# karenyang/GCN-VAE

Measured on AMD Instinct MI355X. Metric: edges/sec R-GCN forward+backward, FB15k-237 emb=200, higher is better.
Workload: dtype f32; 1 GPU; FB15k-237-shaped synthetic full graph (BASELINE configs[1]): 14541 entities, 474 directed relation types, E=544230 directed edges on this rank (544230 in the trained graph), 2-layer R-GCN-VAE bdd num_bases=100 emb_dim=200 dropout 0.2, 0 IAF blocks, DistMult decoder on T=220000 triplets per rank, step = fwd + loss(BCE+reg+KL+MMD) + bwd + clip + Adam; edges_per_gpu=544230, trained_graph_edges=544230, nodes=14541, triplets_per_gpu=220000, n_flows=0, gemm_precision=f32, launch=hipgraph, parallelism=single GPU, optimizer=replicated clip + Adam, k1_operands=f32

## Files before the change

gcn-vae_amd/csrc/k_loss.hip:

```cpp
#include "common.h"

namespace gv {

constexpr int RED_BLOCKS = 1024;

__device__ __forceinline__ float block_sum_256(float v, float* sm ) {
    v = wave_sum(v);
    const int lane = threadIdx.x & 63, w = threadIdx.x >> 6;
    __syncthreads();
    if (lane == 0) sm[w] = v;
    __syncthreads();
    return sm[0] + sm[1] + sm[2] + sm[3];
}

__global__ __launch_bounds__(256) void k_final_sum(const float* part, int n, float scale, float* out, int accumulate) {
    __shared__ float sm[4];
    float acc = 0.f;
    for (int i = threadIdx.x; i < n; i += 256) acc += part[i];
    const float tot = block_sum_256(acc, sm);
    if (threadIdx.x == 0) *out = accumulate ? *out + scale * tot : scale * tot;
}

__global__ __launch_bounds__(256) void k_loss_combine(const float* p0, int n0, float s0, const float* p1, int n1, float s1,
                                                      const float* p2, int n2, float s2, const float* p3, int n3, float s3,
// ... 1019 lines not shown
    for (int i = blockIdx.x * 256 + threadIdx.x; i < total; i += gridDim.x * 256) {
        const int j = i / h, c = i - j * h;
        const float raw = z_pre[(size_t)(k + j) * h + c];
        const float v = softplus_t(raw) + 1e-8f;
        float gm = 0.f, gs = 0.f;
        for (int r = j; r < s; r += k) {
            gm += g[(size_t)r * h + c];
            gs += g[(size_t)r * h + c] * eps[(size_t)r * h + c];
        }
        const float gr = gs * 0.5f / sqrtf(v) * (raw > 20.f ? 1.f : 1.f / (1.f + expf(-raw)));
        gz_pre[i] = accumulate ? gz_pre[i] + gm : gm;
        gz_pre[total + i] = accumulate ? gz_pre[total + i] + gr : gr;
    }
}

struct DmFusedParams {
    const int4* items;
    int n_items;
    const int* rel_s;
    const int* rel_o;
    const int* rel_tid;
    const float* e;
    int ld_e;
    const float* w;
    int ld_w;
    const float* labels;
    const float* bias;
    const int* pos3;
    float* score;
    float* delta;
// ... 518 lines not shown
extern "C" int gv_prior_sample_fwd(const float* z_pre, const float* eps, float* out, int s, int k, int h, void* stream) {
    GV_REQUIRE(z_pre && eps && out, GV_ERR_NULL, "gv_prior_sample_fwd: NULL pointer");
    GV_REQUIRE(s > 0 && k > 0 && h > 0, GV_ERR_SHAPE, "gv_prior_sample_fwd: bad shape");
    hipLaunchKernelGGL(k_prior_sample_fwd, dim3((s * h + 255) / 256), dim3(256), 0, GV_ST, z_pre, eps, out, s, k, h);
    return launch_status("gv_prior_sample_fwd");
}

extern "C" int gv_prior_sample_bwd(const float* z_pre, const float* eps, const float* g, float* gz_pre, int accumulate,
                                   int s, int k, int h, void* stream) {
    GV_REQUIRE(z_pre && eps && g && gz_pre, GV_ERR_NULL, "gv_prior_sample_bwd: NULL pointer");
    GV_REQUIRE(s > 0 && k > 0 && h > 0, GV_ERR_SHAPE, "gv_prior_sample_bwd: bad shape");
    hipLaunchKernelGGL(k_prior_sample_bwd, dim3((k * h + 255) / 256), dim3(256), 0, GV_ST, z_pre, eps, g, gz_pre, accumulate, s, k, h);
    return launch_status("gv_prior_sample_bwd");
}

extern "C" int gv_distmult_bce_fwd_grad(const int32_t* items, int n_items, const int32_t* rel_s, const int32_t* rel_o,
                                        const int32_t* rel_tid, const float* embed, int ld_e, const float* w_rel, int ld_w,
                                        const float* labels, const float* bias, const int32_t* pos3, float* score,
                                        float* delta, float* u, float* partial, float* workspace, int64_t t, int h,
                                        void* stream) {
    GV_REQUIRE(items && rel_s && rel_o && rel_tid && embed && w_rel && labels && score && delta && u && workspace,
               GV_ERR_NULL, "gv_distmult_bce_fwd_grad: NULL pointer");
    GV_REQUIRE(t > 0 && t < (1ll << 30) && n_items > 0, GV_ERR_SHAPE, "gv_distmult_bce_fwd_grad: t=%lld n_items=%d",
               (long long)t, n_items);
    GV_REQUIRE(h > 0 && h <= 256 && h % 4 == 0 && ld_e >= h && ld_w >= h && ld_e % 4 == 0 && ld_w % 4 == 0, GV_ERR_SHAPE,
               "gv_distmult_bce_fwd_grad: h=%d (ld %d, %d): the fused sweep covers h <= 256, h %% 4 == 0", h, ld_e, ld_w);
    GV_REQUIRE(aligned16(embed) && aligned16(w_rel) && aligned16(u) && aligned16(partial), GV_ERR_ALIGN,
               "gv_distmult_bce_fwd_grad: 16-B alignment required");
    DmFusedParams p{(const int4*)items, n_items, rel_s, rel_o, rel_tid, embed, ld_e, w_rel, ld_w, labels, bias, pos3,
                    score, delta, u, partial, workspace, h};
// ... 27 lines not shown
```

gcn-vae_amd/encoders.py:

```python
import random

import numpy as np
import torch
import torch.nn as nn
import torch.nn.functional as F

from . import ops, prob
from .flows import MADE, PermuteLayer
from .layers import RelGraphConv


class EmbeddingLayer(ops.StayOnDevice, nn.Module):
    def __init__(self, num_nodes, h_dim):
        super().__init__()
        self.embedding = nn.Embedding(num_nodes, h_dim)

    def forward(self, g, h, r, norm):
        h = ops.to_module_device(self.embedding.weight, h)
        return ops.embedding(self.embedding.weight, h.squeeze(), ops.device_rng(self.embedding.weight.device),
                             sole_consumer=True)


class DistLayer(ops.StayOnDevice, nn.Module):

# ... 57 lines not shown
        idx = torch.distributions.categorical.Categorical(self.pi).sample((batch,))
        x = prob.sample_gaussian(m[idx], v[idx])
        if self.n_flows > 0:
            for flow in self.nf[::-1]:
                x, _ = flow.inverse(x)
        return x

    def compute_kernel(self, x, y):
        dim = x.size(1)
        d2 = (x.unsqueeze(1) - y.unsqueeze(0)).pow(2).mean(2) / float(dim)
        return torch.exp(-d2)

    def get_kl(self, z):
        return ops.kl_to_mixture(z, self.z_mean, self.z_sigma, self.z_pre.squeeze(0), self.flow_log_prob)

    def _prior_draw(self, device, dtype):
        num_sample = 200
        rows = (num_sample // self.k) * self.k if num_sample // self.k > 1 else self.k
        if self.mmd_eps_override is not None:
            eps = self.mmd_eps_override
        elif self._prior_eps_next is not None:
            eps, self._prior_eps_next = self._prior_eps_next, None
        else:
            eps = torch.empty(rows, self.h_dim, device=device, dtype=dtype)
            ops.device_rng(device).fill([(eps, ops.RNG_NORMAL, 0.0, self.rng_stream_prior)])
        return ops.prior_sample(self.z_pre.squeeze(0), eps)

    def _prior_rows(self):
        num_sample = 200
        return (num_sample // self.k) * self.k if num_sample // self.k > 1 else self.k

    def _draw_noise(self, n, device):
        jobs, eps = [], self.eps_override
        for layer in (self.rconv_layer_1, self.rconv_layer_2):
            if layer.wants_keep_mask():
                layer._keep_next = torch.empty(n, layer.out_feat, dtype=torch.uint8, device=device)
                jobs.append(layer.keep_job(layer._keep_next))
        if eps is None:
            eps = torch.empty(n, self.h_dim, dtype=torch.float32, device=device)
            jobs.append((eps, ops.RNG_NORMAL, 0.0, self.rng_stream_eps))
        if self.batch_mmd_prior_with_forward and self.training and self.mmd_eps_override is None:
            self._prior_eps_next = torch.empty(self._prior_rows(), self.h_dim, dtype=torch.float32, device=device)
            jobs.append((self._prior_eps_next, ops.RNG_NORMAL, 0.0, self.rng_stream_prior))
        if jobs:
            ops.device_rng(device).fill(jobs)
        return eps

    def mmd_inputs(self, z):
        num_sample = 200
        if self._z_pri_flowed is not None:
            z_pri, self._z_pri_flowed = self._z_pri_flowed, None
        else:
            z_pri = self._prior_draw(z.device, z.dtype)
            if self.n_flows > 0:
                for flow in self.nf:
                    z_pri, _ = flow.forward(z_pri)
        if self.mmd_index_override is not None:
            pick = self.mmd_index_override
        elif self.row_part is not None and getattr(self.row_part, 'real_positions', None) is not None:
            real = self.row_part.real_positions
            pick = torch.as_tensor(real[random.sample(range(len(real)), num_sample)], device=z.device)
        else:
            pick = torch.tensor(random.sample(range(z.shape[0]), num_sample), device=z.device)
        return z_pri, pick

    def get_mmd(self, z):
        z_pri, pick = self.mmd_inputs(z)
        return ops.mmd(z_pri, ops.embedding(z, pick))
# ... 176 lines not shown
```

gcn-vae_amd/lib.py:

```python
import ctypes
import os

import torch

_HERE = os.path.dirname(os.path.abspath(__file__))
LIB_PATH = os.path.join(_HERE, 'libgcnvae_hip.so')

_P, _I, _L, _F = ctypes.c_void_p, ctypes.c_int, ctypes.c_int64, ctypes.c_float

SIGNATURES = {
    'gv_version': (_I, []),
    'gv_last_error_string': (ctypes.c_char_p, []),
    'gv_index_caps': (None, [_L, _I, _I, _P, _P, _P]),
    'gv_index_workspace_bytes': (_L, [_L, _I]),
    'gv_build_csr': (_I, [_P, _L, _I, _I, _P, _P, _P, _I, _P, _I, _P, _L, _P]),
    'gv_build_csr_batch_workspace_bytes': (_L, [_P, _I]),
    'gv_build_csr_batch': (_I, [_P, _I, _P, _L, _P]),
    'gv_triplet_lists': (_I, [_P, _I, _L, _P, _P, _P, _P, _P, _P, _P, _P, _P]),
    'gv_widen2_i32': (_I, [_P, _P, _L, _P, _P, _L, _P]),
    'gv_graph_index_build': (_I, [_P, _P, _L, _I, _I, _I, _I, _P, _P, _P, _P, _I, _P, _I, _P, _P, _P, _P, _I, _P, _I, _P, _L, _P]),
    'gv_relation_index_build': (_I, [_P, _P, _P, _P, _P, _L, _I, _I, _P, _P, _P, _P, _P, _P, _P, _I, _P, _I, _P, _L, _P]),
    'gv_triplet_index_build': (_I, [_P, _L, _I, _I, _I, _I, _P, _P, _P, _P, _P, _I, _P, _I, _P, _P, _P, _P, _P, _I, _P, _I,
                                    _P, _L, _P]),
    'gv_perm_sample': (_I, [_L, _L, ctypes.c_uint64, ctypes.c_uint64, _P, _P, ctypes.c_uint32, _P, _P]),
# ... 126 lines not shown
    'gv_mean_sq2': (_I, [_P, _L, _F, _P, _L, _F, _P, _P, _P, _L, _P]),
    'gv_axpby': (_I, [_L, _P, _F, _P, _F, _P, _P]),
    'gv_mul': (_I, [_L, _P, _P, _P, _P]),
    'gv_mul_multi': (_I, [_I, _P, _P, _P, _P, _P]),
    'gv_kl_workspace_bytes': (_L, [_L, _I, _I]),
    'gv_kl_fwd': (_I, [_P, _P, _I, _P, _P, _P, _P, _P, _P, _L, _I, _I, _P, _P]),
    'gv_kl_bwd': (_I, [_P, _P, _I, _P, _P, _P, _P, _F, _F, _P, _P, _P, _P, _I, _P, _I, _L, _I, _I, _P, _P]),
    'gv_reparam_kl_fwd': (_I, [_P, _P, _P, _P, _P, _P, _P, _P, _L, _I, _I, _P]),
    'gv_reparam_kl_bwd': (_I, [_P, _P, _P, _P, _P, _P, _P, _F, _F, _P, _P, _P, _I, _P, _L, _I, _I, _P]),
    'gv_loss_combine': (_I, [_P, _L, _P, _L, _L, _P, _L, _I, _I, _P, _I, _I, _F, _F, _F, _P, _P, _P, _P]),
    'gv_lincomb4': (_I, [_P, _F, _P, _F, _P, _F, _P, _F, _P, _P]),
    'gv_mmd_fwd': (_I, [_P, _P, _P, _I, _I, _I, _P, _P, _P]),
    'gv_mmd_bwd': (_I, [_P, _P, _P, _I, _I, _I, _P, _F, _P, _P, _P]),
    'gv_prior_sample_fwd': (_I, [_P, _P, _P, _I, _I, _I, _P]),
    'gv_prior_sample_bwd': (_I, [_P, _P, _P, _P, _I, _I, _I, _I, _P]),
    'gv_iaf_update_fwd': (_I, [_P, _P, _I, _P, _P, _P, _L, _I, _P]),
    'gv_iaf_update_bwd': (_I, [_P, _P, _I, _P, _P, _P, _P, _P, _P, _L, _I, _P]),
    'gv_iaf_update_bwd_acc': (_I, [_P, _P, _I, _P, _P, _P, _P, _I, _P, _P, _L, _I, _P]),
    'gv_rowsum': (_I, [_P, _I, _I, _I, _P, _L, _P]),
    'gv_reverse_cols': (_I, [_P, _P, _L, _I, _P]),
    'gv_mean_rows_multi': (_I, [_I, _P, _L, _P, _P, _P, _P]),
    'gv_mean_rows_bwd': (_I, [_P, _L, _L, _P, _P, _P]),
    'gv_adam_step': (_I, [_P, _P, _P, _P, _L, _P, _F, _F, _F, _F, _F, _P, _P]),
    'gv_clip_adam_step': (_I, [_P, _P, _P, _P, _L, _P, _P, _F, _F, _F, _F, _F, _P, _I, _P]),
}

_lib = None
_fns = {}


# ... 61 lines not shown
```

gcn-vae_amd/ops.py:

```python
import contextlib
import ctypes as _ct
import itertools as _it
import os as _os
from dataclasses import dataclass
from typing import Optional

import torch

from . import lib
from .lib import ptr

ACT_NONE, ACT_RELU = 0, 1

DIRECT_GRAD = {}
GRAD_FRESH = set()
DIRECT_EPOCH = [0]


def _stamp_direct(ctx):
    ctx._gv_direct_epoch = DIRECT_EPOCH[0]


def _verify_direct(ctx):
    if getattr(ctx, '_gv_direct_epoch', DIRECT_EPOCH[0]) != DIRECT_EPOCH[0]:
# ... 2533 lines not shown
        z_pre, eps = ctx.saved_tensors
        if g is None:
            return None, None
        g = _chk(g.contiguous(), name='g')
        d_zp = _direct_flat(z_pre)
        gz = d_zp if d_zp is not None else torch.empty_like(z_pre)
        lib.call('gv_prior_sample_bwd', ptr(z_pre), ptr(eps), ptr(g), ptr(gz), 1 if d_zp is not None else 0, eps.shape[0],
                 z_pre.shape[0] // 2, z_pre.shape[1], lib.stream())
        return (None if d_zp is not None else gz), None


def prior_sample(z_pre, eps):
    return _PriorSample.apply(z_pre, eps)


class _LossHead(torch.autograd.Function):

    @staticmethod
    def forward(ctx, z, z_mean, z_sigma, w_rel, z_pre, flp, z_pri, pick, labels, tidx, reg_w, kl_w, mmd_w, score_bias,
                embed_rows=None, rows_dev=None, kl_link=None, grad_mode=True):
        z, ld_z = _row_major(z, 'embed')
        if rows_dev is not None:
            rows_dev = _chk(rows_dev.reshape(-1), torch.int32, 'rows_dev')
            if kl_w <= 0 or embed_rows is not None:
                raise NotImplementedError('rows_dev needs kl_w > 0 (the padding rows are masked in the KL pass) and no embed_rows')
        w_rel, ld_w = _row_major(w_rel, 'w_relation')
        labels = _chk(labels.reshape(-1), name='labels')
        dev, (n, h), T = z.device, z.shape, tidx.T
        if labels.numel() != T:
            raise ValueError('labels / triplets length mismatch')
        f32 = dict(dtype=torch.float32, device=dev)
        ctx.set_materialize_grads(False)
        scal = torch.empty(4, **f32)
        pred, reg, kl, mmd = scal[0:1], scal[1:2], scal[2:3], scal[3:4]
        ws, ws2 = torch.empty(2048, **f32), torch.empty(1024, **f32)
        score = torch.empty(T, **f32)
        loss = torch.empty((), **f32)
        bias = flp if (score_bias and flp is not None) else None
        resp = wsk = z_post = wsm = None
        link = kl_link if (kl_link is not None and not kl_link.claimed and kl_w > 0 and flp is None and rows_dev is None
                           and embed_rows is None and kl_link.matches(z_pre) and kl_link.resp.shape[0] == n) else None
        if link is not None:
            link.claimed = True
        if kl_w > 0:
            z_mean, z_sigma = _chk(z_mean.contiguous(), name='z_mean'), _chk(z_sigma.contiguous(), name='z_sigma')
            z_pre = _chk(z_pre.contiguous(), name='z_pre')
            k = z_pre.shape[0] // 2
            if link is None:
                wsk = torch.empty(int(lib.load().gv_kl_workspace_bytes(n, h, k)) // 4, **f32)
                resp = torch.empty(n, k, **f32)
        if mmd_w > 0:
            z_pri = _chk(z_pri.contiguous(), name='z_pri')
            pick = _chk(pick.reshape(-1), torch.int64, 'pick')
            wsm = torch.empty(z_pri.shape[0] + pick.numel(), **f32)
        if ld_z != h or ld_w != h:
            raise ValueError('loss_head needs contiguous embeddings and relation table')
        st = lib.stream()
        if link is not None:
            resp, wsk = link.resp, link.ws
        elif kl_w > 0:
            lib.call('gv_kl_fwd', ptr(z), ptr(z_mean), h, ptr(z_sigma), ptr(z_pre), ptr(flp), ptr(resp), None, ptr(wsk),
                     n, h, k, ptr(rows_dev), st)
        if mmd_w > 0:
            lib.call('gv_mmd_fwd', ptr(z_pri), ptr(z), ptr(pick), z_pri.shape[0], pick.numel(), h, None, ptr(wsm), st)
        z_count = z.numel() if embed_rows is None else int(embed_rows) * h
        lib.call('gv_mean_sq2', ptr(z), z.numel(), 1.0 / z_count, ptr(w_rel), w_rel.numel(), 1.0 / w_rel.numel(), None,
                 ptr(ws2), ptr(rows_dev), n, st)
        ctx.fused = None
        if grad_mode and (ctx.needs_input_grad[0] or ctx.needs_input_grad[3]) and distmult_fused_ok(z, ld_z, w_rel, ld_w):
            ctx.fused = _distmult_fused_fwd(z, ld_z, w_rel, ld_w, labels, bias, tidx, score, ws)
            ctx.ws = ws
        else:
            lib.call('gv_distmult_bce_fwd', ptr(z), ld_z, ptr(w_rel), ld_w, ptr(tidx.trip32), ptr(tidx.fwd_order), ptr(labels),
                     ptr(bias), ptr(score), None, ptr(ws), T, h, st)
        lib.call('gv_loss_combine', ptr(ws), T, ptr(ws2), z.numel(), w_rel.numel(), ptr(wsk) if kl_w > 0 else None, n, h,
                 (z_pre.shape[0] // 2) if kl_w > 0 else 0, ptr(wsm) if mmd_w > 0 else None,
                 z_pri.shape[0] if mmd_w > 0 else 0, pick.numel() if mmd_w > 0 else 0, float(reg_w), float(kl_w),
                 float(mmd_w), ptr(scal), ptr(loss), ptr(rows_dev), st)
        ctx.save_for_backward(z, z_mean if kl_w > 0 else None, z_sigma if kl_w > 0 else None, w_rel,
                              z_pre if kl_w > 0 else None, resp, z_pri if mmd_w > 0 else None, z_post,
                              pick if mmd_w > 0 else None, labels, score, wsk, rows_dev)
        ctx.meta = (tidx, float(reg_w), float(kl_w), float(mmd_w), bias is not None, flp is not None and kl_w > 0)
        ctx.z_count = z_count
        ctx.kl_link = link
        ctx.direct_w = _direct(w_rel) if ld_w == h else None
        _stamp_direct(ctx)
        out_pred, out_kl, out_mmd = pred.reshape(()), kl.reshape(1), mmd.reshape(())
        ctx.mark_non_differentiable(out_pred, out_kl, out_mmd)
        return loss, out_pred, out_kl, out_mmd

    @staticmethod
    def backward(ctx, g, _gp, _gk, _gm):
        if g is None:
            return (None,) * 18
        z, z_mean, z_sigma, w_rel, z_pre, resp, z_pri, z_post, pick, labels, score, wsk, rows_dev = ctx.saved_tensors
        z_count = ctx.z_count
        tidx, reg_w, kl_w, mmd_w, has_bias, flp_in_kl = ctx.meta
        dev, (n, h), T = z.device, z.shape, tidx.T
        f32 = dict(dtype=torch.float32, device=dev)
        g = _chk(g.reshape(1).contiguous(), name='gloss')
        fused = ctx.fused
        dscore = torch.empty(T, **f32) if fused is None else None
        dbias = torch.empty((), **f32) if has_bias else None
        ws = torch.empty(1024, **f32) if fused is None else None
        link = ctx.kl_link
        gz = torch.empty_like(z) if link is None else None
        gm = gv = gzp = d_zp = g_pri = g_post = None
        if link is not None:
            link.gkl, link.gscale, link.z_extra = g, kl_w, 2.0 * reg_w / z_count
            d_zp = True
        elif kl_w > 0:
            k = z_pre.shape[0] // 2
            d_zp = _direct_flat(z_pre)
            gm, gv = torch.empty_like(z), torch.empty_like(z)
            gzp = d_zp if d_zp is not None else torch.empty_like(z_pre)
        if mmd_w > 0:
            g_pri = torch.empty_like(z_pri)
        _verify_direct(ctx)
        d_w = ctx.direct_w
        g_w = d_w if d_w is not None else torch.empty_like(w_rel)
        g_flp = torch.empty((), **f32) if (has_bias or flp_in_kl) else None
        st = lib.stream()
        with fork(1):
            s1 = lib.stream()
            if link is not None:
                pass
            elif kl_w > 0:
                lib.call('gv_kl_bwd', ptr(z), ptr(z_mean), h, ptr(z_sigma), ptr(z_pre), ptr(resp), ptr(g), kl_w,
                         2.0 * reg_w / z_count, ptr(gz), ptr(gm), ptr(gv), ptr(gzp), 1 if d_zp is not None else 0, ptr(wsk),
                         1, n, h, k, ptr(rows_dev), s1)
            else:
                lib.call('gv_axpby', z.numel(), ptr(g), 2.0 * reg_w / z_count, ptr(z), 0.0, ptr(gz), s1)
            if mmd_w > 0 and link is None:
                lib.call('gv_mmd_bwd', ptr(z_pri), ptr(z), ptr(pick), z_pri.shape[0], pick.numel(), h, ptr(g), mmd_w,
                         ptr(g_pri), ptr(gz), s1)
        if fused is not None:
            d_inc = _distmult_fused_finish(fused, g, tidx, w_rel, h, 2.0 * reg_w / w_rel.numel(), g_w, d_w is not None, ctx.ws,
                                           dbias)
            idx_inc = None if tidx.pos3 is not None else tidx.inc_tid
        else:
            if tidx.pos3 is not None:
                d_inc, d_rel, idx_inc, idx_rel = torch.empty(2 * T, **f32), torch.empty(T, **f32), None, None
            else:
                d_inc, d_rel, idx_inc, idx_rel = dscore, dscore, tidx.inc_tid, tidx.rel_tid
            lib.call('gv_bce_grad', ptr(score), ptr(labels), ptr(g), ptr(dscore), ptr(tidx.pos3),
                     ptr(d_inc) if tidx.pos3 is not None else None, ptr(d_rel) if tidx.pos3 is not None else None,
                     ptr(dbias), ptr(ws), T, st)
            bdd_grad_weight(tidx.rel, tidx.rel_s, tidx.rel_o, d_rel, idx_rel, z, z, h, 1, 1, out=g_w,
                            accumulate=d_w is not None)
            lib.call('gv_axpby', w_rel.numel(), ptr(g), 2.0 * reg_w / w_rel.numel(), ptr(w_rel), 1.0, ptr(g_w), st)
        join(1)
        g_z = bdd_aggregate(indices.largest_first(tidx.inc) if indices.K1_ITEMS_LARGEST_FIRST else tidx.inc, tidx.inc_other, tidx.inc_rel,
                            d_inc, idx_inc, z, w_rel, h, 1, 1, addend=gz)
        if link is not None and mmd_w > 0:
            lib.call('gv_mmd_bwd', ptr(z_pri), ptr(z), ptr(pick), z_pri.shape[0], pick.numel(), h, ptr(g), mmd_w,
                     ptr(g_pri), ptr(g_z), st)
        if g_flp is not None:
            lib.call('gv_lincomb4', ptr(dbias) if has_bias else None, 1.0, ptr(g) if flp_in_kl else None, kl_w, None, 0.0,
                     None, 0.0, ptr(g_flp), st)
        return (g_z, gm, gv, (None if d_w is not None else g_w), (None if d_zp is not None else gzp), g_flp, g_pri, None,
                None, None, None, None, None, None, None, None, None, None)


def loss_head(z, z_mean, z_sigma, w_rel, z_pre, flp, z_pri, pick, labels, tidx, reg_w, kl_w, mmd_w, score_bias,
              embed_rows=None, rows_dev=None):
    return _LossHead.apply(z, z_mean, z_sigma, w_rel, z_pre, flp, z_pri, pick, labels, tidx, float(reg_w), float(kl_w),
                           float(mmd_w), bool(score_bias), embed_rows, rows_dev, getattr(z, '_gv_kl_link', None),
                           torch.is_grad_enabled())


from .made import *
from .made import _ChainLayer, _RowLayer, _MADEForward, _MADEForwardBF16
from . import made


TRANSE_MAX_DIM = 512


def _i32(t, name, n=None):
    t = _chk(t, torch.int32, name)
    if not t.is_contiguous() or (n is not None and t.numel() != n):
        raise ValueError(f'{name}: expected a contiguous int32 tensor of {n} entries')
    return t
# ... 364 lines not shown
```

gcn-vae_amd/train.py:

```python
import argparse
import time

import numpy as np
import torch
import torch.nn as nn

from . import ops, ranking, sampling
from .optim import FlatAdam
from .data import load_data
from .encoders import KGVAE, RGCN
from .sampling import node_norm_to_edge_norm


class LinkPredict(ops.StayOnDevice, nn.Module):
    def __init__(self, model_class, in_dim, h_dim, num_rels, num_bases=-1, num_hidden_layers=1, dropout=0,
                 use_cuda=True, reg_param=0, kl_param=0, mmd_param=0, k=1, n_flows=0):
        super().__init__()
        self.encoder = model_class(num_nodes=in_dim, h_dim=h_dim, out_dim=h_dim, num_rels=num_rels * 2,
                                   num_bases=num_bases, num_hidden_layers=num_hidden_layers, dropout=dropout,
                                   use_self_loop=use_cuda, use_cuda=use_cuda, k=k, n_flows=n_flows)
        self.reg_param, self.kl_param, self.mmd_param = reg_param, kl_param, mmd_param
        if kl_param > 0 and hasattr(self.encoder, 'fuse_kl_with_reparam'):
            self.encoder.fuse_kl_with_reparam = True
        if mmd_param > 0 and hasattr(self.encoder, 'batch_mmd_prior_with_forward'):
# ... 16 lines not shown
        return ops.distmult_score(embedding, self.w_relation, self.triplet_index(embedding, triplets))

    def forward(self, g, h, r, norm):
        return self.encoder.forward(g, h, r, norm)

    def regularization_loss(self, embedding):
        return ops.mean_sq(embedding) + ops.mean_sq(self.w_relation)

    def get_loss(self, g, embed, triplets, labels):
        enc = self.encoder
        tidx = self.triplet_index(embed, triplets)
        vae = isinstance(enc, KGVAE)
        flp = enc.get_flow_log_prob() if vae else None
        kl_w = self.kl_param if vae else 0.0
        mmd_w = self.mmd_param if vae else 0.0
        z_pri, pick = enc.mmd_inputs(embed) if mmd_w > 0 else (None, None)
        part = getattr(enc, 'row_part', None) if vae else None
        if part is not None:
            return self._get_loss_rows(part, embed, tidx, flp, kl_w, mmd_w, z_pri, pick, labels)
        loss, predict_loss, kl, mmd = ops.loss_head(
            embed, enc.z_mean if kl_w > 0 else None, enc.z_sigma if kl_w > 0 else None, self.w_relation,
            enc.z_pre.squeeze(0) if kl_w > 0 else None, flp, z_pri, pick, labels, tidx, self.reg_param, kl_w, mmd_w,
            score_bias=self.n_flows > 0, rows_dev=getattr(self, 'rows_dev', None))
        kl = kl.reshape(()) if kl_w > 0 else kl.reshape(1)
        mmd = mmd.reshape(()) if mmd_w > 0 else mmd.reshape(1)
        if kl_w <= 0 or mmd_w <= 0:
            loss = loss.reshape(1)
        return loss, predict_loss, kl, mmd


def _get_loss_rows(self, part, embed, tidx, flp, kl_w, mmd_w, z_pri, pick, labels):
# ... 427 lines not shown
```

include/gcnvae.h:

```cpp
#ifndef GCNVAE_H
#define GCNVAE_H

#include <stdint.h>

#ifdef __cplusplus
extern "C" {
#endif

typedef enum {
    GV_OK = 0,
    GV_ERR_NULL = -1,
    GV_ERR_SHAPE = -2,
    GV_ERR_ALIGN = -3,
    GV_ERR_WORKSPACE = -4
} gv_status;

enum { GV_ACT_NONE = 0, GV_ACT_RELU = 1 };

int gv_version(void);
const char* gv_last_error_string(void);

int gv_segment_items_count(const int32_t* rowptr, int n_seg, int chunk, int32_t* n_chunks, int32_t* n_slots,
                           int32_t* is_split, void* stream);
int gv_segment_items_fill(const int32_t* rowptr, int n_seg, int chunk, const int32_t* item_off,
// ... 391 lines not shown
                      int accumulate_zpre, float* workspace, int64_t n, int h, int k, void* stream);

int gv_loss_combine(const float* ws_pred, int64_t t, const float* ws_reg, int64_t n_embed, int64_t n_wrel,
                    const float* ws_kl, int64_t n_nodes, int h, int k, const float* ws_mmd, int sx, int sy, float reg_w,
                    float kl_w, float mmd_w, float* scal , float* loss, const int32_t* rows_dev,
                    void* stream);
int gv_lincomb4(const float* a0, float c0, const float* a1, float c1, const float* a2, float c2, const float* a3,
                float c3, float* out, void* stream);
int gv_mmd_fwd(const float* x, const float* y, const int64_t* y_index, int sx, int sy, int h, float* mmd, float* workspace,
               void* stream);
int gv_mmd_bwd(const float* x, const float* y, const int64_t* y_index, int sx, int sy, int h, const float* gmmd, float gscale,
               float* gx, float* gy, void* stream);
int gv_prior_sample_fwd(const float* z_pre, const float* eps, float* out, int s, int k, int h, void* stream);
int gv_prior_sample_bwd(const float* z_pre, const float* eps, const float* g, float* gz_pre, int accumulate, int s, int k,
                        int h, void* stream);

int gv_iaf_update_fwd(const float* z, const float* net, int ld_net, const float* x_old, const int32_t* colcount,
                      float* x_new, int64_t n, int d, void* stream);
int gv_iaf_update_bwd(const float* z, const float* net, int ld_net, const int32_t* colcount, const float* g_xnew,
                      const float* g_logdet , float* g_z, float* g_net, float* g_xold, int64_t n, int d,
                      void* stream);
int gv_iaf_update_bwd_acc(const float* z, const float* net, int ld_net, const int32_t* colcount, const float* g_xnew,
                          const float* g_logdet, float* g_z, int gz_accumulate, float* g_net, float* g_xold, int64_t n, int d,
                          void* stream);
int gv_rowsum(const float* x, int ld, int col0, int ncols, float* out, int64_t n, void* stream);
int gv_reverse_cols(const float* x, float* out, int64_t n, int d, void* stream);
int gv_mean_rows_multi(int count, const float* const* x, int64_t n, const int32_t* rows_dev, float* out, float* workspace,
                       void* stream);
int gv_mean_rows_bwd(const float* g, int64_t len, int64_t n, const int32_t* rows_dev, float* out, void* stream);

// ... 71 lines not shown
```

Before: 576.1 million edges/s.

## Fuse prior sampling into MMD kernels and cache kernel matrix for backward

Adds a forward kernel that draws the mixture-prior samples in place (means and softplus scales staged in LDS) and computes the MMD Gaussian kernel sums. It also stores the full kernel matrix for reuse. A new backward kernel reads that stored matrix instead of recomputing exponentials, and folds the prior-sample backward into the same pass, writing z_pre gradients directly. The goal is fewer launches and less redundant work in the MMD term, at the cost of extra memory traffic for the kernel matrix and more complex LDS-heavy kernels.

```diff
diff --git a/gcn-vae_amd/csrc/k_loss.hip b/gcn-vae_amd/csrc/k_loss.hip
--- a/gcn-vae_amd/csrc/k_loss.hip
+++ b/gcn-vae_amd/csrc/k_loss.hip
@@ -1057,6 +1057,314 @@
     }
 }
 
+constexpr int MT_R = 2;
+constexpr int MT_NG = 4 * MMD_WAVES;
+
+template <int G>
+struct MtRows {
+    const float* mix;
+    const float* eps;
+    const float* z;
+    const int64_t* pick;
+    int kh, k, h;
+    bool on[G];
+    int cl[G];
+
+    __device__ __forceinline__ void prior(int r, float4 (&v)[G]) const {
+        const int j = r % k;
+        float4 e4[G];
+#pragma unroll
+        for (int g = 0; g < G; ++g) e4[g] = *reinterpret_cast<const float4*>(eps + (size_t)r * h + cl[g]);
+#pragma unroll
+        for (int g = 0; g < G; ++g) {
+            const float4 m4 = *reinterpret_cast<const float4*>(mix + j * h + cl[g]);
+            const float4 s4 = *reinterpret_cast<const float4*>(mix + kh + j * h + cl[g]);
+            const float4 t = make_float4(m4.x + e4[g].x * s4.x, m4.y + e4[g].y * s4.y, m4.z + e4[g].z * s4.z, m4.w + e4[g].w * s4.w);
+            v[g] = on[g] ? t : make_float4(0.f, 0.f, 0.f, 0.f);
+        }
+    }
+    __device__ __forceinline__ const float* post_ptr(int j) const { return z + (size_t)pick[j] * h; }
+    __device__ __forceinline__ void post(const float* p, float4 (&v)[G]) const {
+#pragma unroll
+        for (int g = 0; g < G; ++g) {
+            const float4 t = *reinterpret_cast<const float4*>(p + cl[g]);
+            v[g] = on[g] ? t : make_float4(0.f, 0.f, 0.f, 0.f);
+        }
+    }
+};
+
+template <int G, bool PRIOR>
+__device__ __forceinline__ void mt_sweep(const MtRows<G>& rows, const float4 (&av)[MT_R][G], int n_live, int nb, float wt, float inv,
+                                         float* krow, int ld, int grp, int l16, float (&tot)[MT_R]) {
+    for (int p0 = 0; p0 < nb; p0 += 2 * MT_NG) {
+        float4 b[2][G];
+        const int pa = min(p0 + grp, nb - 1), pb = min(p0 + MT_NG + grp, nb - 1);
+        if (PRIOR) {
+            rows.prior(pa, b[0]);
+            rows.prior(pb, b[1]);
+        } else {
+            const float* ra = rows.post_ptr(pa);
+            const float* rb = rows.post_ptr(pb);
+            rows.post(ra, b[0]);
+            rows.post(rb, b[1]);
+        }
+#pragma unroll
+        for (int u = 0; u < 2; ++u) {
+            const int p = p0 + u * MT_NG + grp;
+#pragma unroll
+            for (int q = 0; q < MT_R; ++q) {
+                const float kv = expf(-row16_sum(mmd_d2_4<G>(av[q], b[u])) * inv);
+                if (p < nb && q < n_live) {
+                    tot[q] += wt * kv;
+                    if (l16 == 0) krow[(size_t)q * ld + p] = kv;
+                }
+            }
+        }
+    }
+}
+
+template <int G>
+__global__ __launch_bounds__(64 * MMD_WAVES) void k_mmd_prior_fwd(const float* z_pre, const float* eps, const float* z,
+                                                                   const int64_t* pick, int s, int sy, int k, int h,
+                                                                   float* z_pri, float* kmat, float* part) {
+    extern __shared__ __attribute__((aligned(16))) float sm[];
+    const int lane = threadIdx.x & 63, l16 = lane & 15;
+    const int grp = (int)(threadIdx.x >> 4);
+    const int kh = k * h;
+    float* red = sm + 2 * kh;
+    const int ntx = (s + MT_R - 1) / MT_R;
+    const bool is_x = (int)blockIdx.x < ntx;
+    const int row0 = (is_x ? (int)blockIdx.x : (int)blockIdx.x - ntx) * MT_R;
+    const int n_own = is_x ? s : sy;
+    const int n_live = min(MT_R, n_own - row0);
+    MtRows<G> rows{sm, eps, z, pick, kh, k, h, {}, {}};
+#pragma unroll
+    for (int g = 0; g < G; ++g) {
+        const int col = 4 * (l16 + 16 * g);
+        rows.on[g] = col < h;
+        rows.cl[g] = rows.on[g] ? col : 0;
+    }
+    if (is_x) {
+        for (int i = threadIdx.x; i < kh; i += 64 * MMD_WAVES) {
+            sm[i] = z_pre[i];
+            sm[kh + i] = sqrtf(softplus_t(z_pre[kh + i]) + 1e-8f);
+        }
+        __syncthreads();
+    }
+    float4 av[MT_R][G];
+#pragma unroll
+    for (int q = 0; q < MT_R; ++q) {
+        const int r = row0 + min(q, n_live - 1);
+        if (is_x) {
+            rows.prior(r, av[q]);
+            if (grp == q && q < n_live) {
+#pragma unroll
+                for (int g = 0; g < G; ++g)
+                    if (rows.on[g]) *reinterpret_cast<float4*>(z_pri + (size_t)r * h + rows.cl[g]) = av[q][g];
+            }
+        } else {
+            rows.post(rows.post_ptr(r), av[q]);
+        }
+    }
+    const float inv = 1.f / ((float)h * (float)h);
+    const float w_same = 1.f / ((float)n_own * (float)n_own), w_xy = -2.f / ((float)s * (float)sy);
+    float* kxx = kmat;
+    float* kyy = kmat + (size_t)s * s;
+    float* kxy = kyy + (size_t)sy * sy;
+    float tot[MT_R];
+#pragma unroll
+    for (int q = 0; q < MT_R; ++q) tot[q] = 0.f;
+    if (is_x) {
+        mt_sweep<G, true>(rows, av, n_live, s, w_same, inv, kxx + (size_t)row0 * s, s, grp, l16, tot);
+        mt_sweep<G, false>(rows, av, n_live, sy, w_xy, inv, kxy + (size_t)row0 * sy, sy, grp, l16, tot);
+    } else {
+        mt_sweep<G, false>(rows, av, n_live, sy, w_same, inv, kyy + (size_t)row0 * sy, sy, grp, l16, tot);
+    }
+    if (l16 == 0) {
+#pragma unroll
+        for (int q = 0; q < MT_R; ++q) red[q * MT_NG + grp] = tot[q];
+    }
+    __syncthreads();
+    if ((int)threadIdx.x < n_live) {
+        float t = 0.f;
+        for (int i = 0; i < MT_NG; ++i) t += red[threadIdx.x * MT_NG + i];
+        part[(is_x ? 0 : s) + row0 + threadIdx.x] = t;
+    }
+}
+
+constexpr int MB_R = 10;
+constexpr int MB_LW = 32;
+constexpr int MB_NPH = MMD_WAVES * (64 / MB_LW);
+constexpr int MB_PC = 16;
+typedef const float __attribute__((address_space(1)))* mb_gptr;
+static_assert(MB_R % 2 == 0, "the weights are laid out two rows at a time");
+__device__ __forceinline__ int mb_slot(int f, int q, int i, int pp2) { return ((f * (pp2 >> 1) + (i >> 1)) * MB_R + q) * 2 + (i & 1); }
+
+__host__ __device__ inline int mb_pp2(int np) { return (((np + MB_NPH - 1) / MB_NPH) + 1) & ~1; }
+__host__ __device__ inline int mb_rowp_floats(int np) { return 2 * ((np + 1) & ~1); }
+inline size_t mb_lds_bytes(int np) {
+    return ((size_t)mb_rowp_floats(np) + (size_t)MB_NPH * MB_R * mb_pp2(np) + MMD_WAVES * MB_R * 64 + MB_R * MB_LW) * sizeof(float);
+}
+
+__global__ __launch_bounds__(64 * MMD_WAVES) void k_mmd_prior_bwd(const float* __restrict__ z_pre, const float* __restrict__ eps,
+                                                                   const float* __restrict__ z_pri, const float* __restrict__ z,
+                                                                   const int64_t* __restrict__ pick, const float* __restrict__ kmat,
+                                                                   int s, int sy, int k, int h, const float* __restrict__ gmmd,
+                                                                   float gscale, float* gz, float* gz_pre, int accumulate) {
+    extern __shared__ __attribute__((aligned(16))) float sm[];
+    const int np = s + sy;
+    const int pp = (np + MB_NPH - 1) / MB_NPH, pp2 = mb_pp2(np);
+    unsigned long long* rowp = reinterpret_cast<unsigned long long*>(sm);
+    float* wk = sm + mb_rowp_floats(np);
+    float* red = wk + MB_NPH * MB_R * pp2;
+    float* grow = red + MMD_WAVES * MB_R * 64;
+    const int tid = threadIdx.x, lane = tid & 63, l32 = lane & (MB_LW - 1);
+    const int w = __builtin_amdgcn_readfirstlane(tid >> 6);
+    const int nsl = (h + MB_LW - 1) / MB_LW, cs = (h + nsl - 1) / nsl;
+    const int unit = (int)blockIdx.x / nsl, slice = (int)blockIdx.x - unit * nsl;
+    const int c = slice * cs + l32;
+    const bool ok = l32 < cs && c < h;
+    const int cc = min(c, h - 1);
+    const bool prior = unit < k;
+    const float inv = 1.f / ((float)h * (float)h);
+    const float gg = gscale * (gmmd ? *gmmd : 1.f);
+    const float n_same = prior ? (float)s : (float)sy;
+    const float c_same = gg * (-2.f * inv) * 2.f / (n_same * n_same);
+    const float c_other = gg * (-2.f * inv) * (-2.f) / ((float)s * (float)sy);
+    const float* kxx = kmat;
+    const float* kyy = kmat + (size_t)s * s;
+    const float* kxy = kyy + (size_t)sy * sy;
+    for (int p = tid; p < np; p += 64 * MMD_WAVES) rowp[p] = reinterpret_cast<unsigned long long>(p < s ? z_pri + (size_t)p * h : z + (size_t)pick[p - s] * h);
+    for (int e = tid; e < MB_NPH * MB_R * pp2; e += 64 * MMD_WAVES) wk[e] = 0.f;
+    const int first = prior ? unit : (unit - k) * MB_R;
+    const int step = prior ? k : 1;
+    const int n_rows = prior ? (first < s ? (s - first + k - 1) / k : 0) : min(MB_R, sy - first);
+    const int pb = (2 * w + (lane >> 5)) * pp;
+    const float4* wstep = reinterpret_cast<const float4*>(wk + (size_t)(2 * w + (lane >> 5)) * MB_R * pp2);
+    float gm = 0.f, gs = 0.f;
+    auto partner = [&](int p) -> float { return reinterpret_cast<mb_gptr>(rowp[min(p, np - 1)])[cc]; };
+    for (int r0 = 0; r0 < n_rows; r0 += MB_R) {
+        const int nr = min(MB_R, n_rows - r0);
+        const int rowb = first + r0 * step;
+        __syncthreads();
+        float a[MB_R], ev[MB_R], acc[MB_R], bv[MB_PC];
+#pragma unroll
+        for (int q = 0; q < MB_R; ++q) {
+            const int row = rowb + min(q, nr - 1) * step;
+            acc[q] = 0.f;
+            a[q] = prior ? z_pri[(size_t)row * h + cc] : z[(size_t)pick[row] * h + cc];
+            ev[q] = prior ? eps[(size_t)row * h + cc] : 0.f;
+        }
+#pragma unroll
+        for (int u = 0; u < MB_PC; ++u) bv[u] = partner(pb + u);
+        constexpr int NT = 64 * MMD_WAVES;
+        {
+            const float* kx = prior ? kxx + (size_t)rowb * s : kxy + rowb;
+            const size_t rs = prior ? (size_t)step * s : 1, ps = prior ? 1 : (size_t)sy;
+            const int d = prior ? s : MB_R;
+            const float cf = prior ? c_same : c_other;
+            for (int e0 = tid; e0 < s * MB_R; e0 += 4 * NT) {
+                float kv[4];
+                int slot[4];
+#pragma unroll
+                for (int u = 0; u < 4; ++u) {
+                    const int e = min(e0 + u * NT, s * MB_R - 1);
+                    const int hi = e / d, lo = e - hi * d;
+                    const int q = prior ? hi : lo, pq = prior ? lo : hi;
+                    kv[u] = kx[min(q, nr - 1) * rs + pq * ps];
+                    const int f = pq / pp;
+                    slot[u] = e0 + u * NT < s * MB_R ? mb_slot(f, q, pq - f * pp, pp2) : -1;
+                    if (q >= nr) slot[u] = -2 - slot[u];
+                }
+#pragma unroll
+                for (int u = 0; u < 4; ++u) {
+                    if (slot[u] >= 0) wk[slot[u]] = cf * kv[u];
+                    else if (slot[u] < -1) wk[-2 - slot[u]] = 0.f;
+                }
+            }
+        }
+        {
+            const float* ky = (prior ? kxy : kyy) + (size_t)rowb * sy;
+            const size_t rs = prior ? (size_t)step * sy : (size_t)sy;
+            const float cf = prior ? c_other : c_same;
+            for (int e0 = tid; e0 < sy * MB_R; e0 += 4 * NT) {
+                float kv[4];
+                int slot[4];
+#pragma unroll
+                for (int u = 0; u < 4; ++u) {
+                    const int e = min(e0 + u * NT, sy * MB_R - 1);
+                    const int q = e / sy, j = e - q * sy, pq = s + j;
+                    kv[u] = ky[min(q, nr - 1) * rs + j];
+                    const int f = pq / pp;
+                    slot[u] = e0 + u * NT < sy * MB_R ? mb_slot(f, q, pq - f * pp, pp2) : -1;
+                    if (q >= nr) slot[u] = -2 - slot[u];
+                }
+#pragma unroll
+                for (int u = 0; u < 4; ++u) {
+                    if (slot[u] >= 0) wk[slot[u]] = cf * kv[u];
+                    else if (slot[u] < -1) wk[-2 - slot[u]] = 0.f;
+                }
+            }
+        }
+        __syncthreads();
+        for (int c0 = 0; c0 < pp2; c0 += MB_PC) {
+            if (c0 > 0) {
+#pragma unroll
+                for (int u = 0; u < MB_PC; ++u) bv[u] = partner(pb + c0 + u);
+            }
+#pragma unroll
+            for (int u = 0; u < MB_PC; u += 2) {
+                if (c0 + u < pp2) {
+                    float4 wv[MB_R / 2];
+#pragma unroll
+                    for (int j = 0; j < MB_R / 2; ++j) wv[j] = wstep[((c0 + u) >> 1) * (MB_R / 2) + j];
+#pragma unroll
+                    for (int j = 0; j < MB_R / 2; ++j) {
+                        acc[2 * j] = fmaf(wv[j].x, a[2 * j] - bv[u], acc[2 * j]);
+                        acc[2 * j] = fmaf(wv[j].y, a[2 * j] - bv[u + 1], acc[2 * j]);
+                        acc[2 * j + 1] = fmaf(wv[j].z, a[2 * j + 1] - bv[u], acc[2 * j + 1]);
+                        acc[2 * j + 1] = fmaf(wv[j].w, a[2 * j + 1] - bv[u + 1], acc[2 * j + 1]);
+                    }
+                }
+            }
+        }
+#pragma unroll
+        for (int q = 0; q < MB_R; ++q) red[(w * MB_R + q) * 64 + lane] = acc[q];
+        __syncthreads();
+        if (w < nr && lane < MB_LW) {
+            float t = 0.f;
+#pragma unroll
+            for (int i = 0; i < MMD_WAVES; ++i) {
+                t += red[(i * MB_R + w) * 64 + lane];
+                t += red[(i * MB_R + w) * 64 + MB_LW + lane];
+            }
+            if (prior) grow[w * MB_LW + lane] = t;
+            else if (ok) atomicAdd(gz + (size_t)pick[rowb + w] * h + c, t);
+        }
+        if (prior) {
+            __syncthreads();
+            if (w == 0 && lane < MB_LW && ok) {
+#pragma unroll
+                for (int q = 0; q < MB_R; ++q) {
+                    if (q < nr) {
+                        const float g = grow[q * MB_LW + lane];
+                        gm += g;
+                        gs += g * ev[q];
+                    }
+                }
+            }
+        }
+    }
+    if (prior && w == 0 && lane < MB_LW && ok) {
+        const size_t i = (size_t)unit * h + c, total = (size_t)k * h;
+        const float raw = z_pre[total + i];
+        const float v = softplus_t(raw) + 1e-8f;
+        const float gr = gs * 0.5f / sqrtf(v) * (raw > 20.f ? 1.f : 1.f / (1.f + expf(-raw)));
+        gz_pre[i] = accumulate ? gz_pre[i] + gm : gm;
+        gz_pre[total + i] = accumulate ? gz_pre[total + i] + gr : gr;
+    }
+}
+
 struct DmFusedParams {
     const int4* items;
     int n_items;
@@ -1605,6 +1913,39 @@
     return launch_status("gv_prior_sample_bwd");
 }
 
+constexpr int MT_MAX_KH = 8064;
+
+extern "C" int gv_mmd_prior_fwd(const float* z_pre, const float* eps, const float* z, const int64_t* pick, int s, int sy, int k,
+                                int h, float* z_pri, float* kmat, float* workspace, void* stream) {
+    GV_REQUIRE(z_pre && eps && z && pick && z_pri && kmat && workspace, GV_ERR_NULL, "gv_mmd_prior_fwd: NULL pointer");
+    GV_REQUIRE(s > 0 && sy > 0 && k > 0 && h > 0 && h <= 256 && h % 4 == 0 && s + sy <= RED_BLOCKS && (int64_t)k * h <= MT_MAX_KH,
+               GV_ERR_SHAPE, "gv_mmd_prior_fwd: s=%d sy=%d k=%d h=%d (need h <= 256, h %% 4 == 0, s+sy <= %d, k*h <= %d)", s, sy, k,
+               h, RED_BLOCKS, MT_MAX_KH);
+    GV_REQUIRE(aligned16(z_pre) && aligned16(eps) && aligned16(z) && aligned16(z_pri), GV_ERR_ALIGN,
+               "gv_mmd_prior_fwd: 16-B alignment required");
+    const int nb = (s + MT_R - 1) / MT_R + (sy + MT_R - 1) / MT_R;
+    const size_t lds = (2 * (size_t)k * h + MT_R * MT_NG) * sizeof(float);
+    hipLaunchKernelGGL(k_mmd_prior_fwd<4>, dim3(nb), dim3(64 * MMD_WAVES), lds, GV_ST, z_pre, eps, z, pick, s, sy, k, h, z_pri, kmat,
+                       workspace);
+    return launch_status("gv_mmd_prior_fwd");
+}
+
+extern "C" int gv_mmd_prior_bwd(const float* z_pre, const float* eps, const float* z_pri, const float* z, const int64_t* pick,
+                                const float* kmat, int s, int sy, int k, int h, const float* gmmd, float gscale, float* gz,
+                                float* gz_pre, int accumulate, void* stream) {
+    GV_REQUIRE(z_pre && eps && z_pri && z && pick && kmat && gz && gz_pre, GV_ERR_NULL, "gv_mmd_prior_bwd: NULL pointer");
+    GV_REQUIRE(s > 0 && sy > 0 && k > 0 && h > 0 && h <= 256 && h % 4 == 0 && s + sy <= RED_BLOCKS, GV_ERR_SHAPE,
+               "gv_mmd_prior_bwd: s=%d sy=%d k=%d h=%d (need h <= 256, h %% 4 == 0, s+sy <= %d)", s, sy, k, h, RED_BLOCKS);
+    const int nsl = (h + MB_LW - 1) / MB_LW;
+    const int nb = (k + (sy + MB_R - 1) / MB_R) * nsl;
+    const size_t lds = mb_lds_bytes(s + sy);
+    static unsigned long long lds_done = 0;
+    if (!raise_dynamic_lds((const void*)k_mmd_prior_bwd, (int)mb_lds_bytes(RED_BLOCKS), lds_done, "gv_mmd_prior_bwd")) return GV_ERR_SHAPE;
+    hipLaunchKernelGGL(k_mmd_prior_bwd, dim3(nb), dim3(64 * MMD_WAVES), lds, GV_ST, z_pre, eps, z_pri, z, pick, kmat, s, sy, k, h,
+                       gmmd, gscale, gz, gz_pre, accumulate);
+    return launch_status("gv_mmd_prior_bwd");
+}
+
 extern "C" int gv_distmult_bce_fwd_grad(const int32_t* items, int n_items, const int32_t* rel_s, const int32_t* rel_o,
                                         const int32_t* rel_tid, const float* embed, int ld_e, const float* w_rel, int ld_w,
                                         const float* labels, const float* bias, const int32_t* pos3, float* score,
diff --git a/gcn-vae_amd/encoders.py b/gcn-vae_amd/encoders.py
--- a/gcn-vae_amd/encoders.py
+++ b/gcn-vae_amd/encoders.py
@@ -95,7 +95,7 @@
     def get_kl(self, z):
         return ops.kl_to_mixture(z, self.z_mean, self.z_sigma, self.z_pre.squeeze(0), self.flow_log_prob)
 
-    def _prior_draw(self, device, dtype):
+    def _prior_draw(self, device, dtype, deferred=False):
         num_sample = 200
         rows = (num_sample // self.k) * self.k if num_sample // self.k > 1 else self.k
         if self.mmd_eps_override is not None:
@@ -105,6 +105,8 @@
         else:
             eps = torch.empty(rows, self.h_dim, device=device, dtype=dtype)
             ops.device_rng(device).fill([(eps, ops.RNG_NORMAL, 0.0, self.rng_stream_prior)])
+        if deferred:
+            return ops.PriorDraw(self.z_pre.squeeze(0), eps)
         return ops.prior_sample(self.z_pre.squeeze(0), eps)
 
     def _prior_rows(self):
@@ -127,12 +129,12 @@
             ops.device_rng(device).fill(jobs)
         return eps
 
-    def mmd_inputs(self, z):
+    def mmd_inputs(self, z, deferred=False):
         num_sample = 200
         if self._z_pri_flowed is not None:
             z_pri, self._z_pri_flowed = self._z_pri_flowed, None
         else:
-            z_pri = self._prior_draw(z.device, z.dtype)
+            z_pri = self._prior_draw(z.device, z.dtype, deferred=deferred and self.n_flows == 0)
             if self.n_flows > 0:
                 for flow in self.nf:
                     z_pri, _ = flow.forward(z_pri)
diff --git a/gcn-vae_amd/lib.py b/gcn-vae_amd/lib.py
--- a/gcn-vae_amd/lib.py
+++ b/gcn-vae_amd/lib.py
@@ -164,6 +164,8 @@
     'gv_mmd_bwd': (_I, [_P, _P, _P, _I, _I, _I, _P, _F, _P, _P, _P]),
     'gv_prior_sample_fwd': (_I, [_P, _P, _P, _I, _I, _I, _P]),
     'gv_prior_sample_bwd': (_I, [_P, _P, _P, _P, _I, _I, _I, _I, _P]),
+    'gv_mmd_prior_fwd': (_I, [_P, _P, _P, _P, _I, _I, _I, _I, _P, _P, _P, _P]),
+    'gv_mmd_prior_bwd': (_I, [_P, _P, _P, _P, _P, _P, _I, _I, _I, _I, _P, _F, _P, _P, _I, _P]),
     'gv_iaf_update_fwd': (_I, [_P, _P, _I, _P, _P, _P, _L, _I, _P]),
     'gv_iaf_update_bwd': (_I, [_P, _P, _I, _P, _P, _P, _P, _P, _P, _L, _I, _P]),
     'gv_iaf_update_bwd_acc': (_I, [_P, _P, _I, _P, _P, _P, _P, _I, _P, _P, _L, _I, _P]),
diff --git a/gcn-vae_amd/ops.py b/gcn-vae_amd/ops.py
--- a/gcn-vae_amd/ops.py
+++ b/gcn-vae_amd/ops.py
@@ -2571,11 +2571,31 @@
     return _PriorSample.apply(z_pre, eps)
 
 
+class PriorDraw:
+
+    def __init__(self, z_pre, eps):
+        self.z_pre, self.eps = z_pre, eps
+
+    def sample(self):
+        return prior_sample(self.z_pre, self.eps)
+
+
+MMD_TILES = _os.environ.get('GV_MMD_TILES', '1') == '1'
+MMD_TILES_MAX_KH = 8064
+MMD_TILES_MAX_ROWS = 1024
+
+
+def mmd_tiles_ok(draw, sy, mmd_w, embed_rows=None):
+    (k2, h), s = draw.z_pre.shape, draw.eps.shape[0]
+    return (MMD_TILES and mmd_w > 0 and embed_rows is None and h % 4 == 0 and h <= 256 and (k2 // 2) * h <= MMD_TILES_MAX_KH
+            and s + sy <= MMD_TILES_MAX_ROWS and draw.eps.shape[1] == h)
+
+
 class _LossHead(torch.autograd.Function):
 
     @staticmethod
     def forward(ctx, z, z_mean, z_sigma, w_rel, z_pre, flp, z_pri, pick, labels, tidx, reg_w, kl_w, mmd_w, score_bias,
-                embed_rows=None, rows_dev=None, kl_link=None, grad_mode=True):
+                embed_rows=None, rows_dev=None, kl_link=None, grad_mode=True, pri_zpre=None, pri_eps=None):
         z, ld_z = _row_major(z, 'embed')
         if rows_dev is not None:
             rows_dev = _chk(rows_dev.reshape(-1), torch.int32, 'rows_dev')
@@ -2594,7 +2614,8 @@
         score = torch.empty(T, **f32)
         loss = torch.empty((), **f32)
         bias = flp if (score_bias and flp is not None) else None
-        resp = wsk = z_post = wsm = None
+        resp = wsk = z_post = wsm = kmat = None
+        tiles = pri_zpre is not None
         link = kl_link if (kl_link is not None and not kl_link.claimed and kl_w > 0 and flp is None and rows_dev is None
                            and embed_rows is None and kl_link.matches(z_pre) and kl_link.resp.shape[0] == n) else None
         if link is not None:
@@ -2607,8 +2628,14 @@
                 wsk = torch.empty(int(lib.load().gv_kl_workspace_bytes(n, h, k)) // 4, **f32)
                 resp = torch.empty(n, k, **f32)
         if mmd_w > 0:
-            z_pri = _chk(z_pri.contiguous(), name='z_pri')
             pick = _chk(pick.reshape(-1), torch.int64, 'pick')
+            if tiles:
+                pri_zpre, pri_eps = _chk(pri_zpre.contiguous(), name='z_pre'), _chk(pri_eps.contiguous(), name='eps')
+                s_pri, s_post = pri_eps.shape[0], pick.numel()
+                z_pri = torch.empty_like(pri_eps)
+                kmat = torch.empty(s_pri * s_pri + s_post * s_post + s_pri * s_post, **f32)
+            else:
+                z_pri = _chk(z_pri.contiguous(), name='z_pri')
             wsm = torch.empty(z_pri.shape[0] + pick.numel(), **f32)
         if ld_z != h or ld_w != h:
             raise ValueError('loss_head needs contiguous embeddings and relation table')
@@ -2618,7 +2645,10 @@
         elif kl_w > 0:
             lib.call('gv_kl_fwd', ptr(z), ptr(z_mean), h, ptr(z_sigma), ptr(z_pre), ptr(flp), ptr(resp), None, ptr(wsk),
                      n, h, k, ptr(rows_dev), st)
-        if mmd_w > 0:
+        if mmd_w > 0 and tiles:
+            lib.call('gv_mmd_prior_fwd', ptr(pri_zpre), ptr(pri_eps), ptr(z), ptr(pick), z_pri.shape[0], pick.numel(),
+                     pri_zpre.shape[0] // 2, h, ptr(z_pri), ptr(kmat), ptr(wsm), st)
+        elif mmd_w > 0:
             lib.call('gv_mmd_fwd', ptr(z_pri), ptr(z), ptr(pick), z_pri.shape[0], pick.numel(), h, None, ptr(wsm), st)
         z_count = z.numel() if embed_rows is None else int(embed_rows) * h
         lib.call('gv_mean_sq2', ptr(z), z.numel(), 1.0 / z_count, ptr(w_rel), w_rel.numel(), 1.0 / w_rel.numel(), None,
@@ -2636,7 +2666,8 @@
                  float(mmd_w), ptr(scal), ptr(loss), ptr(rows_dev), st)
         ctx.save_for_backward(z, z_mean if kl_w > 0 else None, z_sigma if kl_w > 0 else None, w_rel,
                               z_pre if kl_w > 0 else None, resp, z_pri if mmd_w > 0 else None, z_post,
-                              pick if mmd_w > 0 else None, labels, score, wsk, rows_dev)
+                              pick if mmd_w > 0 else None, labels, score, wsk, rows_dev, kmat,
+                              pri_zpre if tiles else None, pri_eps if tiles else None)
         ctx.meta = (tidx, float(reg_w), float(kl_w), float(mmd_w), bias is not None, flp is not None and kl_w > 0)
         ctx.z_count = z_count
         ctx.kl_link = link
@@ -2649,8 +2680,10 @@
     @staticmethod
     def backward(ctx, g, _gp, _gk, _gm):
         if g is None:
-            return (None,) * 18
-        z, z_mean, z_sigma, w_rel, z_pre, resp, z_pri, z_post, pick, labels, score, wsk, rows_dev = ctx.saved_tensors
+            return (None,) * 20
+        (z, z_mean, z_sigma, w_rel, z_pre, resp, z_pri, z_post, pick, labels, score, wsk, rows_dev, kmat, pri_zpre,
+         pri_eps) = ctx.saved_tensors
+        tiles = kmat is not None
         z_count = ctx.z_count
         tidx, reg_w, kl_w, mmd_w, has_bias, flp_in_kl = ctx.meta
         dev, (n, h), T = z.device, z.shape, tidx.T
@@ -2662,7 +2695,7 @@
         ws = torch.empty(1024, **f32) if fused is None else None
         link = ctx.kl_link
         gz = torch.empty_like(z) if link is None else None
-        gm = gv = gzp = d_zp = g_pri = g_post = None
+        gm = gv = gzp = d_zp = g_pri = g_post = gzp_pri = d_zp_pri = None
         if link is not None:
             link.gkl, link.gscale, link.z_extra = g, kl_w, 2.0 * reg_w / z_count
             d_zp = True
@@ -2671,9 +2704,21 @@
             d_zp = _direct_flat(z_pre)
             gm, gv = torch.empty_like(z), torch.empty_like(z)
             gzp = d_zp if d_zp is not None else torch.empty_like(z_pre)
-        if mmd_w > 0:
+        if mmd_w > 0 and tiles:
+            d_zp_pri = _direct_flat(pri_zpre)
+            gzp_pri = d_zp_pri if d_zp_pri is not None else torch.empty_like(pri_zpre)
+        elif mmd_w > 0:
             g_pri = torch.empty_like(z_pri)
         _verify_direct(ctx)
+
+        def mmd_bwd(gz_into, stream):
+            if tiles:
+                lib.call('gv_mmd_prior_bwd', ptr(pri_zpre), ptr(pri_eps), ptr(z_pri), ptr(z), ptr(pick), ptr(kmat),
+                         z_pri.shape[0], pick.numel(), pri_zpre.shape[0] // 2, h, ptr(g), mmd_w, ptr(gz_into), ptr(gzp_pri),
+                         1 if d_zp_pri is not None else 0, stream)
+            else:
+                lib.call('gv_mmd_bwd', ptr(z_pri), ptr(z), ptr(pick), z_pri.shape[0], pick.numel(), h, ptr(g), mmd_w,
+                         ptr(g_pri), ptr(gz_into), stream)
         d_w = ctx.direct_w
         g_w = d_w if d_w is not None else torch.empty_like(w_rel)
         g_flp = torch.empty((), **f32) if (has_bias or flp_in_kl) else None
@@ -2689,8 +2734,7 @@
             else:
                 lib.call('gv_axpby', z.numel(), ptr(g), 2.0 * reg_w / z_count, ptr(z), 0.0, ptr(gz), s1)
             if mmd_w > 0 and link is None:
-                lib.call('gv_mmd_bwd', ptr(z_pri), ptr(z), ptr(pick), z_pri.shape[0], pick.numel(), h, ptr(g), mmd_w,
-                         ptr(g_pri), ptr(gz), s1)
+                mmd_bwd(gz, s1)
         if fused is not None:
             d_inc = _distmult_fused_finish(fused, g, tidx, w_rel, h, 2.0 * reg_w / w_rel.numel(), g_w, d_w is not None, ctx.ws,
                                            dbias)
@@ -2710,20 +2754,26 @@
         g_z = bdd_aggregate(indices.largest_first(tidx.inc) if indices.K1_ITEMS_LARGEST_FIRST else tidx.inc, tidx.inc_other, tidx.inc_rel,
                             d_inc, idx_inc, z, w_rel, h, 1, 1, addend=gz)
         if link is not None and mmd_w > 0:
-            lib.call('gv_mmd_bwd', ptr(z_pri), ptr(z), ptr(pick), z_pri.shape[0], pick.numel(), h, ptr(g), mmd_w,
-                     ptr(g_pri), ptr(g_z), st)
+            mmd_bwd(g_z, st)
         if g_flp is not None:
             lib.call('gv_lincomb4', ptr(dbias) if has_bias else None, 1.0, ptr(g) if flp_in_kl else None, kl_w, None, 0.0,
                      None, 0.0, ptr(g_flp), st)
         return (g_z, gm, gv, (None if d_w is not None else g_w), (None if d_zp is not None else gzp), g_flp, g_pri, None,
-                None, None, None, None, None, None, None, None, None, None)
+                None, None, None, None, None, None, None, None, None, None,
+                (None if d_zp_pri is not None else gzp_pri), None)
 
 
 def loss_head(z, z_mean, z_sigma, w_rel, z_pre, flp, z_pri, pick, labels, tidx, reg_w, kl_w, mmd_w, score_bias,
               embed_rows=None, rows_dev=None):
+    pri_zpre = pri_eps = None
+    if isinstance(z_pri, PriorDraw):
+        if mmd_tiles_ok(z_pri, pick.numel(), float(mmd_w), embed_rows) and z.shape[1] == z_pri.z_pre.shape[1]:
+            pri_zpre, pri_eps, z_pri = z_pri.z_pre, z_pri.eps, None
+        else:
+            z_pri = z_pri.sample()
     return _LossHead.apply(z, z_mean, z_sigma, w_rel, z_pre, flp, z_pri, pick, labels, tidx, float(reg_w), float(kl_w),
                            float(mmd_w), bool(score_bias), embed_rows, rows_dev, getattr(z, '_gv_kl_link', None),
-                           torch.is_grad_enabled())
+                           torch.is_grad_enabled(), pri_zpre, pri_eps)
 
 
 from .made import *
diff --git a/gcn-vae_amd/train.py b/gcn-vae_amd/train.py
--- a/gcn-vae_amd/train.py
+++ b/gcn-vae_amd/train.py
@@ -54,7 +54,7 @@
         flp = enc.get_flow_log_prob() if vae else None
         kl_w = self.kl_param if vae else 0.0
         mmd_w = self.mmd_param if vae else 0.0
-        z_pri, pick = enc.mmd_inputs(embed) if mmd_w > 0 else (None, None)
+        z_pri, pick = enc.mmd_inputs(embed, deferred=True) if mmd_w > 0 else (None, None)
         part = getattr(enc, 'row_part', None) if vae else None
         if part is not None:
             return self._get_loss_rows(part, embed, tidx, flp, kl_w, mmd_w, z_pri, pick, labels)
diff --git a/include/gcnvae.h b/include/gcnvae.h
--- a/include/gcnvae.h
+++ b/include/gcnvae.h
@@ -429,6 +429,11 @@
 int gv_prior_sample_fwd(const float* z_pre, const float* eps, float* out, int s, int k, int h, void* stream);
 int gv_prior_sample_bwd(const float* z_pre, const float* eps, const float* g, float* gz_pre, int accumulate, int s, int k,
                         int h, void* stream);
+int gv_mmd_prior_fwd(const float* z_pre, const float* eps, const float* z, const int64_t* pick, int s, int sy, int k, int h,
+                     float* z_pri, float* kmat, float* workspace, void* stream);
+int gv_mmd_prior_bwd(const float* z_pre, const float* eps, const float* z_pri, const float* z, const int64_t* pick,
+                     const float* kmat, int s, int sy, int k, int h, const float* gmmd, float gscale, float* gz, float* gz_pre,
+                     int accumulate, void* stream);
 
 int gv_iaf_update_fwd(const float* z, const float* net, int ld_net, const float* x_old, const int32_t* colcount,
                       float* x_new, int64_t n, int d, void* stream);
```

After: 581.8 million edges/s (median of 6 runs). 1.01x the previous value.
